# jhollowed/PyTEMDiags

Measured on AMD Instinct MI355X. Metric: grid-points/sec through full TEM pipeline (ncol*nlev*nt), higher is better.
Workload: dtype f64; 1 GPU; ne120 (777602 cols) x 72 lev x 30 snapshots per GPU, L=50, 1-degree zonal grid (M=180), ten GM16 Table-A1 outputs; ncol=777602, nlev=72, nt=30, sweeps=latitude-class, single sweep, mirror_paired_sweeps=True

## Files before the change

include/temx.h:

```cpp
#ifndef TEMX_H
#define TEMX_H

#include <stdint.h>

#ifdef __cplusplus
extern "C" {
#endif

typedef struct temx_plan temx_plan;

enum { TEMX_F64 = 0, TEMX_F32 = 1 };

enum {
  TEMX_OK = 0,
  TEMX_EINVAL = -1,
  TEMX_EHIP = -2,
  TEMX_ENOMEM = -3,
  TEMX_ERANK = -4,
  TEMX_ESTATE = -5,
  TEMX_EUNSUPPORTED = -6,
  TEMX_EINTERNAL = -7
};

enum {
  TEMX_DEFER_FINALIZE = 1,
  TEMX_NO_SYMMETRY = 2,
  TEMX_NO_CLASSES = 4,
  TEMX_NO_QR = 8,
  TEMX_LAT_TOL_F32 = 16
};

enum {
  TEMX_OPT_FORM = 1,
  TEMX_OPT_OS_MAP = 2,
  TEMX_OPT_OP_MAP = 3,
  TEMX_OPT_OS_SUBSAMPLE = 4,
  TEMX_OPT_TRACER_ONE_PASS = 5,
  TEMX_OPT_SINGLE_SWEEP_MIN_GROUPS = 6,
  TEMX_OPT_OS_CONTRACT = 7,
  TEMX_OPT_MISSING = 8,
  TEMX_OPT_MIN_COVERAGE = 9,
  TEMX_OPT_MISSING_WEIGHT = 10
};
enum {
  TEMX_FORM_AUTO = -1,
  TEMX_FORM_TWO_PASS = 0,
  TEMX_FORM_CLASS_SUMS = 1,
  TEMX_FORM_SINGLE_SWEEP = 2,
  TEMX_FORM_NO_SINGLE_SWEEP = 3,
  TEMX_FORM_MASKED = 4
};

enum {
  TEMX_MAT_Y0 = 0,
  TEMX_MAT_Y0P = 1,
  TEMX_MAT_GRAM = 2,
  TEMX_MAT_GINV = 3,
  TEMX_MAT_Y0INV = 4,
  TEMX_MAT_GRAM2 = 5,
  TEMX_MAT_GX = 6,
  TEMX_MAT_GSUB = 7,
  TEMX_MAT_COVERAGE = 8
};

enum {
// ... 135 lines not shown
```

pytemdiags_amd/_lib.py:

```python
from __future__ import annotations

import ctypes as C
import os

_HERE = os.path.dirname(os.path.abspath(__file__))
LIB_PATH = os.environ.get("TEMX_LIB") or os.path.join(_HERE, "libtemx.so")

ABI_VERSION = 402
F64, F32 = 0, 1
DEFER_FINALIZE = 1
NO_SYMMETRY = 2
NO_CLASSES = 4
NO_QR = 8
LAT_TOL_F32 = 16
MAT_Y0, MAT_Y0P, MAT_GRAM, MAT_GINV, MAT_Y0INV, MAT_GRAM2, MAT_GX, MAT_GSUB = 0, 1, 2, 3, 4, 5, 6, 7
MAT_COVERAGE = 8
OPT_FORM, OPT_OS_MAP, OPT_OP_MAP, OPT_OS_SUBSAMPLE, OPT_TRACER_ONE_PASS, OPT_SINGLE_SWEEP_MIN_GROUPS, OPT_OS_CONTRACT = 1, 2, 3, 4, 5, 6, 7
OPT_MISSING, OPT_MIN_COVERAGE, OPT_MISSING_WEIGHT = 8, 9, 10
MISSING_MODES = {"raise": 0, "mask": 1}
FORM_AUTO, FORM_TWO_PASS, FORM_CLASS_SUMS, FORM_SINGLE_SWEEP, FORM_NO_SINGLE_SWEEP = -1, 0, 1, 2, 3
FORM_MASKED = 4
FORMS = {"auto": FORM_AUTO, "two-pass": FORM_TWO_PASS, "class-sums": FORM_CLASS_SUMS,
         "single-sweep": FORM_SINGLE_SWEEP, "no-single-sweep": FORM_NO_SINGLE_SWEEP}

RESULT_NAMES = ("vtem", "omegatem", "wtem", "psitem", "epfy", "epfz", "epdiv",
                "utendepfd", "utendvtem", "utendwtem")
ZONAL_NAMES = ("ub", "vb", "thetab", "wapb", "upvpb", "upwappb", "vptpb", "dub_dp", "dthetab_dp",
               "ubcoslat", "dubcoslat_dlat", "psi", "psicoslat", "dpsicoslat_dlat", "dpsi_dp",
               "int_vbdp")
EDDY_NAMES = ("up", "vp", "thetap", "wapp", "upvp", "upwapp", "vptp")
TRACER_RESULT_NAMES = ("etfy", "etfz", "etdiv", "qtendetfd", "qtendvtem", "qtendwtem")
TRACER_ZONAL_NAMES = ("qb", "qpvpb", "qpwappb", "dqb_dp", "qbcoslat", "dqbcoslat_dlat")
TRACER_EDDY_NAMES = ("qp", "qpvp", "qpwapp")

ERRORS = {0: "TEMX_OK", -1: "TEMX_EINVAL", -2: "TEMX_EHIP", -3: "TEMX_ENOMEM", -4: "TEMX_ERANK",
          -5: "TEMX_ESTATE", -6: "TEMX_EUNSUPPORTED", -7: "TEMX_EINTERNAL"}

_vp, _i, _i64, _dp, _u64 = C.c_void_p, C.c_int, C.c_int64, C.POINTER(C.c_double), C.c_uint64
SIGNATURES = [
    ("temx_version", _i, []),
    ("temx_last_error", C.c_char_p, []),
# ... 100 lines not shown
```

pytemdiags_amd/csrc/kernels_op2.hpp:

```cpp
#pragma once
#include "kernels_op.hpp"

namespace temx {

template <int NA, int NB>
struct OpwSlot {
  double sd[2][NA][64];
  double y[NB * 16];
};

template <int TBS, int NA>
__device__ __forceinline__ void opw_round(const OpwSlot<NA, 2 * TBS>* slots, int par, int t0, int nbw,
                                          uint32_t yoff, int lane, double (&acc)[NA][(TBS + 1) / 2]) {
  asm volatile("s_waitcnt lgkmcnt(0)\n\ts_barrier" ::: "memory");
#pragma unroll
  for (int j = 0; j < 4; ++j) {
    double b[NA];
#pragma unroll
    for (int f = 0; f < NA; ++f) b[f] = slots[j].sd[par][f][lane];
#pragma unroll
    for (int tl = 0; tl < (TBS + 1) / 2; ++tl)
      if (tl < nbw) {
        const double ya = slots[j].y[(t0 + tl) * 16 + yoff];
#pragma unroll
// ... 554 lines not shown
};
template <> struct RowLoad<float> {
  static __device__ __forceinline__ void ld(float& dst, uint32_t voff, uint64_t sbase) {
    asm volatile("global_load_dword %0, %1, %2 " TEMX_ROWLOAD_MOD : "=v"(dst) : "v"(voff), "s"(sbase) : "memory");
  }
};
__device__ __forceinline__ double temx_rcp_count(double n) {
  double r = __builtin_amdgcn_rcp(n);
  return __builtin_fma(__builtin_fma(-n, r, 1.0), r, r);
}
template <int N, typename T>
__device__ __forceinline__ void row_wait(T& a, T& b, T& c, T& d) {
  asm volatile("s_waitcnt vmcnt(%4)" : "+v"(a), "+v"(b), "+v"(c), "+v"(d) : "n"(N) : "memory");
}
template <int N, typename T>
__device__ __forceinline__ void row_wait(T& a, T& b, T& c) {
  asm volatile("s_waitcnt vmcnt(%3)" : "+v"(a), "+v"(b), "+v"(c) : "n"(N) : "memory");
}
template <typename T>
__device__ __forceinline__ void row_touch(T& a) {
  asm volatile("" : "+v"(a)::"memory");
}

template <typename T, int TBS, int TBX, int NBR, int PD, int KIND = 0>
__global__ void __launch_bounds__(256, 1)
sweep_osr_kernel(FieldPtrs<4> fp, int64_t D, int K, int KX, const double* __restrict__ ycx,
                 const int4* __restrict__ crow, const int2* __restrict__ csplit,
                 const double* __restrict__ colscale, const double* __restrict__ rho, int K4,
                 double* __restrict__ px, double* __restrict__ pp, int nsplit, int ndt) {
  using KD = OsKind<KIND>;
  constexpr int NF = KD::NF, NFX = KD::NFX, NP = KD::NP;
  constexpr int NBX = 2 * TBX;
  constexpr int YE = NBX * 16;
  constexpr int YJ = (YE + 255) / 256;
  constexpr int MB = CLS_MB;
  constexpr int NCH = 4;
  constexpr int NV = 2 * (NF + NP);
  constexpr int NPR = KD::NPR, NPL = NP - NPR;
  static_assert(NBR <= TBS && TBS <= TBX, "reference degree <= L <= 2L");
  static_assert(YJ <= 2, "Y quarter per thread");
  static_assert((PD - 1) * CLS_MB * KD::NF + (CLS_MB - 1) * KD::NF + 2 <= 63, "the ring is counted in vmcnt (6 bits)");
  extern __shared__ double lds[];
  int split, dq;
  if (!wg_work((ndt + 3) / 4, nsplit, split, dq)) return;
  const int tid = threadIdx.x;
  const int wave = uniform_wave(), lane = tid & 63;
  const int c = lane & 15, g = lane >> 4;
  const int64_t colr = (int64_t)dq * 64 + lane < D ? (int64_t)dq * 64 + lane : D - 1;
  const uint32_t colb32 = (uint32_t)colr * (uint32_t)sizeof(T);
  const int dt = dq * 4 + wave;
  const int64_t d = (int64_t)dt * 16 + c;
  const bool dvalid = dt < ndt && d < D;
  const int64_t dcl = dvalid ? d : D - 1;
  const int b0 = __builtin_amdgcn_readfirstlane(csplit[split].x);
  const int b1 = __builtin_amdgcn_readfirstlane(csplit[split + 1].x);
  int grp = __builtin_amdgcn_readfirstlane(csplit[split].y);
  const uint32_t aoff_p = (uint32_t)(g * 4 + (lane & 3));
  const uint32_t aoff_r = (uint32_t)((lane & 3) * 4 + g);
  double* ybase = lds;
  double* cn = lds + 2 * YE;
  double* cb = lds + 2 * YE + 16 + wave * (NF * 2 * NBR * 64) + lane;
  double* apl = lds + 2 * YE + 16 + 4 * (NF * 2 * NBR * 64) + wave * (NPL * 2 * TBS * 64) + lane;
  double* ex = lds + 2 * YE + 16 + 4 * (NF * 2 * NBR * 64) + 4 * (NPL * 2 * TBS * 64);
  double* exw = ex + wave * 64 + lane;
  const double* exr = ex + g * 64 + wave * 16 + c;
  const double sth = (KD::TF >= 0 && colscale != nullptr) ? colscale[colr] : 1.0;
#pragma unroll
  for (int i = 0; i < NPL * 2 * TBS; ++i) apl[i * 64] = 0.0;
  double apr[NPR > 0 ? NPR : 1][2 * TBS];
#pragma unroll
  for (int k = 0; k < (NPR > 0 ? NPR : 1); ++k)
#pragma unroll
    for (int t = 0; t < 2 * TBS; ++t) apr[k][t] = 0.0;
#pragma unroll
  for (int f = 0; f < NF; ++f)
#pragma unroll
    for (int tb = 0; tb < 2 * NBR; ++tb) {
      const int l = tb < NBR ? 2 * (4 * tb + g) : 2 * (4 * (tb - NBR) + g) + 1;
      const double v = rho[((int64_t)f * K4 + (l < K ? l : K - 1)) * D + dcl];
      cb[(f * 2 * NBR + tb) * 64] = l < K ? v : 0.0;
    }
  uint64_t fbase[NF];
#pragma unroll
  for (int f = 0; f < NF; ++f) fbase[f] = reinterpret_cast<uint64_t>(fp.p[f]);
  { double sth_ready = sth; asm volatile("" : "+v"(sth_ready)); }

  double ax[NFX][NBX];
#pragma unroll
  for (int f = 0; f < NFX; ++f)
// ... 46 lines not shown
        const int ta = t < TBX ? tp : TBS + tp;
#pragma unroll
        for (int k = 0; k < NPR; ++k) apr[k][ta] = TEMX_MFMA4(ya, dP[k][t < TBX ? 0 : 1], apr[k][ta]);
        if constexpr (NPL > 0) {
          double v[NPL > 0 ? NPL : 1];
#pragma unroll
          for (int k = 0; k < NPL; ++k) v[k] = apl[(k * 2 * TBS + ta) * 64];
#pragma unroll
          for (int k = 0; k < NPL; ++k) v[k] = TEMX_MFMA4(ya, dP[NPR + k][t < TBX ? 0 : 1], v[k]);
#pragma unroll
          for (int k = 0; k < NPL; ++k) apl[(k * 2 * TBS + ta) * 64] = v[k];
        }
      }
    }
  };
  auto park_north = [&]() __attribute__((always_inline)) {
#pragma unroll
    for (int f = 0; f < NF; ++f) { sN[f] = s[f]; x0N[f] = x0[f]; s[f] = 0.0; }
#pragma unroll
    for (int k = 0; k < NP; ++k) { qN[k] = q[k]; q[k] = 0.0; }
    cntN = cnt;
    cnt = 0.0;
  };
  int4 rn;
  auto step = [&](auto posc, int b) __attribute__((always_inline)) {
    constexpr int POS = decltype(posc)::value % NCH;
    constexpr int P = decltype(posc)::value % PD;
    {
      const int4 r1 = rn;
      rn = crow[(int64_t)(b + PD) * 4 + wave];
      issue(std::integral_constant<int, (P + PD - 1) % PD>{}, r1);
    }
    if (left > 0) {
      if (!(TEMX_OS_SKIP & 1)) pending_chunk(std::integral_constant<int, POS>{});
      --left;
    }
    static_assert(NF == 4 || NF == 3, "row_wait has forms for 3 and 4 fields");
    static_for<MB>([&](auto jc) __attribute__((always_inline)) {
      constexpr int j = decltype(jc)::value;
      constexpr int NW = (PD - 1) * MB * NF + (MB - 1 - j) * NF;
      if constexpr (NF == 4) row_wait<NW>(xb[P][j][0], xb[P][j][1], xb[P][j][2], xb[P][j][3]);
      else row_wait<NW>(xb[P][j][0], xb[P][j][1], xb[P][j][2]);
    });
#pragma unroll
    for (int j = 0; j < YJ; ++j) row_touch(ys[j]);
    const int fl = er[P][0] >> 27;
    const bool south = (fl & (CLS_SOUTH << 1)) != 0;
    if ((fl & (CLS_FIRST << 1)) || (south && !prev_south)) {
      if (south && north_open) park_north();
      north_open = !south;
#pragma unroll
      for (int f = 0; f < NF; ++f) x0[f] = (double)xb[P][0][f];
    }
    prev_south = south;
#pragma unroll
    for (int j = 0; j < ((TEMX_OS_SKIP & 4) ? 0 : MB); ++j) {
      const double w = er[P][j] < 0 ? 0.0 : 1.0;
      double dx[NF];
#pragma unroll
      for (int f = 0; f < NF; ++f) dx[f] = (double)xb[P][j][f] - x0[f];
#pragma unroll
      for (int f = 0; f < NF; ++f) s[f] += w * dx[f];
#pragma unroll
      for (int k = 0; k < NP; ++k) q[k] += (w * dx[KD::pa(k)]) * dx[KD::pb(k)];
      cnt += w;
    }
    if (fl & (CLS_LAST << 1)) {
      prev_south = false;
      if (north_open) park_north();
      north_open = false;
      if (left > 0)
        static_for<NCH>([&](auto cc) __attribute__((always_inline)) {
          if (((decltype(cc)::value - POS - 1) & (NCH - 1)) < left) pending_chunk(cc);
        });
      const double rnN = cntN > 0.0 ? temx_rcp_count(cntN) : 0.0, rnS = cnt > 0.0 ? temx_rcp_count(cnt) : 0.0;
      double val[NV];
#pragma unroll
      for (int f = 0; f < NF; ++f) {
        const double sc = f == KD::TF ? sth : 1.0;
        val[f] = (sN[f] * rnN + x0N[f]) * sc;
        val[NF + NP + f] = (s[f] * rnS + x0[f]) * sc;
      }
#pragma unroll
      for (int k = 0; k < NP; ++k) {
        const double sc = k == KD::TP ? sth : 1.0;
        val[NF + k] = (qN[k] - sN[KD::pa(k)] * sN[KD::pb(k)] * rnN) * sc;
        val[2 * NF + NP + k] = (q[k] - s[KD::pa(k)] * s[KD::pb(k)] * rnS) * sc;
      }
      if (!(TEMX_OS_SKIP & 8)) asm volatile("s_waitcnt lgkmcnt(0)\n\ts_barrier" ::: "memory");
      ycur ^= 1;
      double* yw = ybase + ycur * YE;
#pragma unroll
      for (int v = 0; v < NV; ++v) exw[v * 256] = val[v];
      if (lane == 0) {
        cn[wave] = cntN;
        cn[4 + wave] = cnt;
      }
#pragma unroll
      for (int j = 0; j < YJ; ++j)
        if (tid + 256 * j < YE) yw[tid + 256 * j] = ys[j];
      if (!(TEMX_OS_SKIP & 8)) asm volatile("s_waitcnt lgkmcnt(0)\n\ts_barrier" ::: "memory");
      ++grp;
      load_ys(grp);
      double m2[2][NF], c2[2][NP];
#pragma unroll
      for (int f = 0; f < NF; ++f) {
        m2[0][f] = exr[f * 256];
        m2[1][f] = exr[(NF + NP + f) * 256];
      }
#pragma unroll
      for (int k = 0; k < NP; ++k) {
        c2[0][k] = exr[(NF + k) * 256];
        c2[1][k] = exr[(2 * NF + NP + k) * 256];
      }
      const double nN = cn[g], nS = cn[4 + g];
      double E[NF], O[NF];
#pragma unroll
      for (int f = 0; f < NF; ++f) E[f] = O[f] = 0.0;
#pragma unroll
      for (int tb = 0; tb < ((TEMX_OS_SKIP & 2) ? 0 : 2 * NBR); ++tb) {
        const int blk = tb < NBR ? tb : TBX + (tb - NBR);
        const double ya = yw[blk * 16 + aoff_r];
#pragma unroll
        for (int f = 0; f < NF; ++f) {
          if (tb < NBR)
            E[f] = TEMX_MFMA4(ya, cb[(f * 2 * NBR + tb) * 64], E[f]);
          else
            O[f] = TEMX_MFMA4(ya, cb[(f * 2 * NBR + tb) * 64], O[f]);
        }
      }
#pragma unroll
      for (int f = 0; f < NF; ++f) {
        m2[0][f] -= E[f] + O[f];
        m2[1][f] -= E[f] - O[f];
      }
#pragma unroll
      for (int f = 0; f < NFX; ++f) {
        const double SNf = nN * m2[0][f], SSf = nS * m2[1][f];
        dS[f][0] = SNf + SSf;
        dS[f][1] = SNf - SSf;
      }
#pragma unroll
      for (int k = 0; k < NP; ++k) {
        const double PNk = c2[0][k] + nN * m2[0][KD::pa(k)] * m2[0][KD::pb(k)];
        const double PSk = c2[1][k] + nS * m2[1][KD::pa(k)] * m2[1][KD::pb(k)];
        dP[k][0] = PNk + PSk;
        dP[k][1] = PNk - PSk;
      }
      yprev = yw;
      left = NCH;
#pragma unroll
      for (int f = 0; f < NF; ++f) s[f] = sN[f] = 0.0;
#pragma unroll
      for (int k = 0; k < NP; ++k) q[k] = qN[k] = 0.0;
      cnt = cntN = 0.0;
    }
  };

  if (b0 < b1) {
    load_ys(grp);
    rn = crow[(int64_t)b0 * 4 + wave];
    static_for<PD - 1>([&](auto kc) __attribute__((always_inline)) {
      constexpr int k = decltype(kc)::value;
      const int4 r0 = rn;
      rn = crow[(int64_t)(b0 + k + 1) * 4 + wave];
      issue(kc, r0);
    });
    constexpr int UNR = PD % 4 == 0 ? PD : PD % 2 == 0 ? 2 * PD : 4 * PD;
    for (int b = b0; b < b1; b += UNR)
      static_for<UNR>([&](auto kc) __attribute__((always_inline)) {
        constexpr int k = decltype(kc)::value;
        if (k == 0 || b + k < b1) step(kc, b + k);
      });
    asm volatile("s_waitcnt vmcnt(0)" ::: "memory");
  }
  if (left > 0) {
    const int first = (b1 - b0) & (NCH - 1);
    static_for<NCH>([&](auto cc) __attribute__((always_inline)) {
      if (((decltype(cc)::value - first) & (NCH - 1)) < left) pending_chunk(cc);
    });
  }
  if (dvalid) {
#pragma unroll
    for (int f = 0; f < NFX; ++f)
#pragma unroll
      for (int t = 0; t < NBX; ++t) {
        const int l = symx_harm<TBX>(t, g);
        if (l < (pp != nullptr ? KX : K4)) px[(((int64_t)split * NFX + f) * KX + l) * D + d] = ax[f][t];
      }
#pragma unroll
    for (int k = 0; k < NP; ++k)
#pragma unroll
      for (int t = 0; t < 2 * TBS; ++t) {
        const int l = sym_harm<TBS>(t, g);
        if (pp != nullptr && l < K) pp[(((int64_t)split * NP + k) * K + l) * D + d] = k < NPR ? apr[k < NPR ? k : 0][t] : apl[((k < NPR ? 0 : k - NPR) * 2 * TBS + t) * 64];
      }
  }
// ... 711 lines not shown
```

pytemdiags_amd/csrc/temx.hip:

```cpp
#include "../../include/temx.h"

#include <hip/hip_runtime.h>

#include <algorithm>
#include <cmath>
#include <cstdarg>
#include <cstdio>
#include <cstdlib>
#include <cstring>
#include <map>
#include <new>
#include <stdexcept>
#include <string>
#include <thread>
#include <atomic>
#include <vector>

#include "kernels.hpp"
#include "kernels_sym.hpp"
#include "kernels_cls.hpp"
#include "kernels_op.hpp"
#include "kernels_op2.hpp"
#include "kernels_osc.hpp"
#include "side_tables.hpp"
// ... 90 lines not shown
  int64_t cgroups = 0, cbatches = 0, ncls = 0;
  int64_t cls_max_side = 0;
  std::vector<int> gbatch0;
  DevBuf crow, ycls;
  std::map<int, DevBuf> csplits;
  Split sp_cproj4, sp_cproj1, sp_ceddy, sp_cflux;
  bool os_built = false, os_on = false;
  bool os_valid = false;
  DevBuf Axq, rho_t;
  int TBX = 0, KX = 0, KR = 0, NQ = 0;
  std::vector<double> h_xc, h_cnt;
  std::vector<int> h_crow;
  std::vector<int> sgbatch0;
  int64_t sgroups = 0, sbatches = 0;
  DevBuf ycx, ycx_s, crow_s, rho, rho0, gaunt , wq2, Gx, Gsinv, Ax , Axs ;
  std::vector<double> h_G_own;
  std::vector<double> h_Gx_own;
  std::vector<double> h_Gx, h_Gs;
  std::vector<double> h_T, h_Ginv, h_G, h_Yq;
  DevBuf oscblk, osAt, osAb, osAtq, osAbq, Bqp;
  OscMats osc{};
  bool osc_lds = false;
  int opt_os_contract = -1;
  int os_keep = 32;
  int64_t tD = 0, tnt = 0, tt0 = 0;
  int opt_form = -1, opt_os_map = -1, opt_op_map = -1, opt_tracer_one_pass = -1, opt_single_sweep_min_groups = -1;
  bool os_tile = false, op_tile = false;
  bool no_qr = false;
  DevBuf side_crow[2][2], side_gfirst[2][2];
  std::map<int, DevBuf> csplits_s;
  Split sp_os, sp_os_s;
  Split sp_copw;
  bool lcls = false, lone = false, xb_valid = false;
  DevBuf ycls_l, pbuf;
  int64_t ycls_lstride = 0;
  Split sp_lflux;
  bool onepass = false, op_valid = false;
  bool c4_valid = false;
  DevBuf csum, ccnt;
  DevBuf Pq;
  DevBuf csq, Pq2;
  bool tq_valid = false;
  DevBuf partial;
  DevBuf opB, opC;
  int opt_missing = 0, opt_min_cov = 500, opt_miss_w = 10;
  bool miss_built = false;
// ... 1442 lines not shown
      static std::atomic<uint64_t> attr_set{0};                                                                     \
      if (int rc_ = lds_attr_once(attr_set, pl->device, reinterpret_cast<const void*>(kern), (int)lds)) return rc_; \
      hipLaunchKernelGGL(kern, grid, block, lds, st, fp, pl->D, pl->K, pl->KX, sub ? pl->ycx_s.d() : pl->ycx.d(),   \
                         static_cast<const int4*>(sub ? pl->crow_s.p : pl->crow.p), cuts, pl->colscale.d(), rho,    \
                         pl->KR, px, pp, sp.nsplit, sp.ndt);                                                        \
      break;                                                                                                        \
    }                                                                                                               \
    if (sizeof(T) == 4) {                 \
      if (pl->cls_max_side > 8 * TEMX_F32_SIDE_CAP)                                                                 \
        return fail(TEMX_EUNSUPPORTED, "single sweep of fp32 fields: a latitude class of this plan has %lld members on one " \
                    "side, and the sweep sums a side in fp32; create the plan with TEMX_LAT_TOL_F32",               \
                    (long long)pl->cls_max_side);                                                                   \
      auto kern = sweep_os2_kernel<float, TBSv, TBXv, NBR, 2, KIND>;                                                \
      const size_t lds = ((size_t)2 * 2 * TBXv * 16 + 16 + (size_t)4 * KD::NF * 2 * NBR * 64 +                      \
                          (size_t)8 * (KD::NP - KD::NPR) * TBSv * 64 + (size_t)(KD::NF + KD::NP) * 512) * 8;        \
      static std::atomic<uint64_t> attr_set{0};                                                                     \
      if (int rc_ = lds_attr_once(attr_set, pl->device, reinterpret_cast<const void*>(kern), (int)lds)) return rc_; \
      const int si = sub ? 1 : 0;                                                                                   \
      hipLaunchKernelGGL(kern, grid, dim3(512), lds, st, fp, pl->D, pl->K, pl->KX, sub ? pl->ycx_s.d() : pl->ycx.d(), \
                         static_cast<const int4*>(pl->side_crow[si][0].p), static_cast<const int4*>(pl->side_crow[si][1].p), \
                         static_cast<const int*>(pl->side_gfirst[si][0].p), static_cast<const int*>(pl->side_gfirst[si][1].p), \
                         cuts, pl->colscale.d(), rho, pl->KR, px, pp, sp.nsplit, sp.ndt);                           \
    } else {                                                                                                        \
      auto kern = sweep_osr_kernel<double, TBSv, TBXv, NBR, 2, KIND>;                                               \
      const size_t lds = ((size_t)2 * 2 * TBXv * 16 + 16 + (size_t)4 * KD::NF * 2 * NBR * 64 +                      \
                          (size_t)4 * (KD::NP - KD::NPR) * 2 * TBSv * 64 + (size_t)2 * (KD::NF + KD::NP) * 256) * 8; \
      static std::atomic<uint64_t> attr_set{0};                                                                     \
      if (int rc_ = lds_attr_once(attr_set, pl->device, reinterpret_cast<const void*>(kern), (int)lds)) return rc_; \
      hipLaunchKernelGGL(kern, grid, block, lds, st, fp, pl->D, pl->K, pl->KX, sub ? pl->ycx_s.d() : pl->ycx.d(),   \
                         static_cast<const int4*>(sub ? pl->crow_s.p : pl->crow.p), cuts, pl->colscale.d(), rho,    \
                         pl->KR, px, pp, sp.nsplit, sp.ndt);                                                        \
    }                                                                                                               \
  } while (0)
  if (pl->TBS == 7 && pl->TBX == 13) TEMX_LOS(7, 13);
  else if (pl->TBS == 4 && pl->TBX == 8) TEMX_LOS(4, 8);
  else if (pl->TBS == 2 && pl->TBX == 4) TEMX_LOS(2, 4);
  else return fail(TEMX_EUNSUPPORTED, "single-sweep form: no instantiation for L = %d", pl->L);
#undef TEMX_LOS
  HIPCHK(hipGetLastError());
  return TEMX_OK;
}

template <int KIND>
static int launch_sweep_os(temx_plan* pl, const FieldPtrs<4>& fp, int dtype, bool sub, const double* rho, double* partial,
                           const Split& sp, hipStream_t st) {
  return dtype == TEMX_F64 ? launch_sweep_os_t<double, KIND>(pl, fp, sub, rho, partial, sp, st)
                           : launch_sweep_os_t<float, KIND>(pl, fp, sub, rho, partial, sp, st);
}

static bool os_supported(const temx_plan* pl) {
  if (!pl->cls || pl->large || pl->weighted || !pl->qbasis || pl->h_crow.empty()) return false;
  const int tbx = (pl->L + 1 + 3) / 4;
  return (pl->TBS == 7 && tbx <= 13) || (pl->TBS == 4 && tbx <= 8) || (pl->TBS == 2 && tbx <= 4);
}
// ... 473 lines not shown
  pl->TB = pl->K <= 16 ? 4 : (pl->K <= 32 ? 8 : (pl->K <= 52 ? 13 : 16));
  pl->stride = pl->TB;
  if (pl->K > 64) {
    pl->large = true;
    pl->nslice = (pl->K + 63) / 64;
    pl->stride = 16 * pl->nslice;
  }
  pl->K4 = 4 * pl->stride;
  pl->M = M;
  pl->lat_out_deg.assign(lat_out_deg_host, lat_out_deg_host + M);
  int rc = TEMX_OK;
  auto bail = [&](int code) {
    temx_plan_destroy(pl);
    return code;
  };

  const double d2r = M_PI / 180.0;
  std::vector<double> xs((size_t)std::max<int64_t>(ncol, M));
  for (int64_t i = 0; i < ncol; ++i) xs[i] = std::cos((90.0 - lat_deg_host[i]) * d2r);
  if ((rc = upload(pl->x, xs.data(), (size_t)ncol * 8))) return bail(rc);
  std::vector<double> norm((size_t)std::max(64, pl->K4), 0.0);
  for (int l = 0; l < pl->K; ++l) norm[l] = std::sqrt((2.0 * l + 1.0) / (4.0 * M_PI));
  if ((rc = upload(pl->norm, norm.data(), norm.size() * 8))) return bail(rc);
  int zero = 0;
  if ((rc = upload(pl->flag, &zero, sizeof(int)))) return bail(rc);

  if ((rc = pl->Y0.ensure((size_t)ncol * pl->K * 8))) return bail(rc);
  if ((rc = pl->yblk.ensure((size_t)(pl->nchunk + 1) * 4 * pl->stride * 16 * 8))) return bail(rc);
  if (hipMemset(pl->yblk.p, 0, pl->yblk.bytes) != hipSuccess) return bail(fail(TEMX_EHIP, "hipMemset of the Y0 blocks failed"));
  if ((rc = build_basis(pl, nullptr, nullptr, pl->Y0.d(), pl->yblk.d()))) return bail(rc);

  for (int m = 0; m < M; ++m) xs[m] = std::cos((90.0 - lat_out_deg_host[m]) * d2r);
  if ((rc = upload(pl->xo, xs.data(), (size_t)M * 8))) return bail(rc);
  if ((rc = pl->Y0p.ensure((size_t)M * pl->K * 8))) return bail(rc);
  if ((rc = pl->Qp.ensure((size_t)M * pl->K * 8))) return bail(rc);
  if ((rc = build_out_basis(pl, nullptr, pl->Y0p.d(), false))) return bail(rc);
  if ((rc = build_out_basis(pl, nullptr, pl->Qp.d(), true))) return bail(rc);

  {
    if ((rc = pl->G.ensure((size_t)pl->K * pl->K * 8))) return bail(rc);
    if ((rc = pl->Ginv.ensure((size_t)pl->K * pl->K * 8))) return bail(rc);
    Split sp = choose_split(pl->K, pl->nchunk, 2 * pl->num_cu);
    if ((rc = pl->partial.ensure((size_t)sp.nsplit * std::min(pl->K, 64) * pl->K * 8))) return bail(rc);
    FieldPtrs<1> fp;
    fp.p[0] = pl->Y0.p;
    if ((rc = project_all<1>(pl, fp, TEMX_F64, pl->K, nullptr, -1, sp, pl->G.d(), 0))) return bail(rc);
    hipError_t e = hipDeviceSynchronize();
    if (e != hipSuccess) return bail(fail(TEMX_EHIP, "gram kernel failed: %s", hipGetErrorString(e)));
// ... 369 lines not shown
struct FormChoice {
  bool two_pass;
  bool force_op;
  int os;
};
static FormChoice form_choice(const temx_plan* pl) {
  FormChoice c{false, false, -1};
  switch (pl->opt_form) {
    case TEMX_FORM_TWO_PASS: c.two_pass = true; c.os = 0; break;
    case TEMX_FORM_CLASS_SUMS: c.force_op = true; c.os = 0; break;
    case TEMX_FORM_SINGLE_SWEEP: c.force_op = true; c.os = 1; break;
    case TEMX_FORM_NO_SINGLE_SWEEP: c.os = 0; break;
    default: break;
  }
  if (const char* e = getenv("TEMX_TWO_PASS")) c.two_pass = e[0] == '1';
  if (const char* e = getenv("TEMX_ONE_PASS")) c.force_op = c.force_op || e[0] == '1';
  if (const char* e = getenv("TEMX_SINGLE_SWEEP")) c.os = e[0] == '0' ? 0 : (e[0] == '1' ? 1 : c.os);
  return c;
}
static bool tile_map(int opt, const char* env) {
  if (const char* e = getenv(env)) return !strcmp(e, "tile");
  return opt == 1;
}
static bool tracer_one_pass_wanted(const temx_plan* pl) {
  if (const char* e = getenv("TEMX_TRACER_ONE_PASS")) return e[0] == '1';
  return pl->opt_tracer_one_pass == 1;
}

int temx_plan_configure(temx_plan* pl, int option, int value) try {
  if (!pl) return fail(TEMX_EINVAL, "null plan");
  switch (option) {
    case TEMX_OPT_FORM:
      if (value < -1 || value > TEMX_FORM_NO_SINGLE_SWEEP) return fail(TEMX_EINVAL, "TEMX_OPT_FORM: unknown form %d", value);
      pl->opt_form = value;
      break;
    case TEMX_OPT_OS_MAP: pl->opt_os_map = value; break;
    case TEMX_OPT_OP_MAP: pl->opt_op_map = value; break;
    case TEMX_OPT_TRACER_ONE_PASS: pl->opt_tracer_one_pass = value; break;
    case TEMX_OPT_OS_SUBSAMPLE:
      if (value < 4) return fail(TEMX_EINVAL, "TEMX_OPT_OS_SUBSAMPLE: at least 4 class-groups");
      if (pl->os_built && value != pl->os_keep) return fail(TEMX_ESTATE, "the single-sweep tables of this plan are built: set the subsample before temx_plan_set_tem");
      pl->os_keep = value;
      break;
    case TEMX_OPT_SINGLE_SWEEP_MIN_GROUPS: pl->opt_single_sweep_min_groups = value; break;
    case TEMX_OPT_OS_CONTRACT: pl->opt_os_contract = value; break;
    case TEMX_OPT_MISSING:
      if (value != 0 && value != 1) return fail(TEMX_EINVAL, "TEMX_OPT_MISSING: 0 (raise) or 1 (mask), got %d", value);
      if (value == 1)
        if (int rc = miss_check(pl)) return rc;
      pl->opt_missing = value;
      pl->miss_valid = false;
      break;
    case TEMX_OPT_MIN_COVERAGE:
      if (value < 0 || value > 1000) return fail(TEMX_EINVAL, "TEMX_OPT_MIN_COVERAGE: per mille in 0..1000, got %d", value);
      pl->opt_min_cov = value;
      break;
    case TEMX_OPT_MISSING_WEIGHT:
      if (value < 4 || value > 14) return fail(TEMX_EINVAL, "TEMX_OPT_MISSING_WEIGHT: tau = 10^-value, value in 4..14, got %d", value);
      pl->opt_miss_w = value;
      break;
    default: return fail(TEMX_EINVAL, "unknown option %d", option);
  }
  pl->tem = false;
  return TEMX_OK;
} TEMX_CATCH

int temx_plan_option(const temx_plan* pl, int option) try {
  if (!pl) return -1;
  switch (option) {
    case TEMX_OPT_FORM:
      if (miss_mode(pl)) return TEMX_FORM_MASKED;
      return pl->os_on ? TEMX_FORM_SINGLE_SWEEP : ((pl->cls && pl->onepass) || (pl->lcls && pl->lone) ? TEMX_FORM_CLASS_SUMS : TEMX_FORM_TWO_PASS);
    case TEMX_OPT_OS_MAP: return tile_map(pl->opt_os_map, "TEMX_OS_MAP") ? 1 : 0;
    case TEMX_OPT_OP_MAP: return tile_map(pl->opt_op_map, "TEMX_OP_MAP") ? 1 : 0;
    case TEMX_OPT_TRACER_ONE_PASS: return tracer_one_pass_wanted(pl) ? 1 : 0;
    case TEMX_OPT_OS_SUBSAMPLE: return pl->os_keep;
    case TEMX_OPT_SINGLE_SWEEP_MIN_GROUPS: return pl->opt_single_sweep_min_groups;
    case TEMX_OPT_OS_CONTRACT: return pl->osc_lds ? 1 : 0;
    case TEMX_OPT_MISSING: return pl->opt_missing;
    case TEMX_OPT_MIN_COVERAGE: return pl->opt_min_cov;
    case TEMX_OPT_MISSING_WEIGHT: return pl->opt_miss_w;
    default: return -1;
  }
} TEMX_CATCH

int temx_plan_set_tem(temx_plan* pl, int nlev, int64_t nt, const double* p_pa_host, double p0) try {
  if (!pl || !p_pa_host) return fail(TEMX_EINVAL, "null argument");
  if (nlev < 2 || nt < 1) return fail(TEMX_EINVAL, "need nlev >= 2 and nt >= 1");
  if ((int64_t)nlev * nt >= ((int64_t)1 << 28)) return fail(TEMX_EINVAL, "nlev*nt must be < 2^28");
  if (pl->M < 2) return fail(TEMX_EINVAL, "need at least 2 zonal-mean latitudes");
  HIPCHK(hipSetDevice(pl->device));
  std::vector<double> p(p_pa_host, p_pa_host + nlev), tab;
  for (int j = 1; j < nlev; ++j)
    if (!(p[j] > p[j - 1])) return fail(TEMX_EINVAL, "pressure must be strictly ascending (front end flips)");
  pl->tem = false;
  pl->onepass = pl->lone = pl->op_valid = pl->xb_valid = pl->tq_valid = false;
  pl->os_on = pl->os_valid = false;
  pl->os_tile = tile_map(pl->opt_os_map, "TEMX_OS_MAP");
  {
    const char* e = getenv("TEMX_OS_CONTRACT");
    pl->osc_lds = e ? !strcmp(e, "lds") : pl->opt_os_contract == 1;
  }
  pl->op_tile = tile_map(pl->opt_op_map, "TEMX_OP_MAP");
  pl->nlev = nlev;
  pl->nt = nt;
  pl->D = (int64_t)nlev * nt;
  pl->tD = pl->D;
  pl->tnt = nt;
  pl->tt0 = 0;
  pl->p0 = p0;
  const int M = pl->M;
  const int64_t D = pl->D;
  int rc;
  if ((rc = upload(pl->p, p.data(), (size_t)nlev * 8))) return rc;
  gradient_table(p, tab);
  if ((rc = upload(pl->pg, tab.data(), tab.size() * 8))) return rc;
  std::vector<double> latr(M), cosl(M), fc(M);
  for (int m = 0; m < M; ++m) {
    const double lat = pl->lat_out_deg[m];
    latr[m] = lat * (M_PI / 180.0);
    cosl[m] = std::cos(lat * M_PI / 180.0);
    fc[m] = 2 * kOm * std::sin(lat * M_PI / 180.0);
  }
  gradient_table(latr, tab);
  if ((rc = upload(pl->lg, tab.data(), tab.size() * 8))) return rc;
  if ((rc = upload(pl->coslat, cosl.data(), (size_t)M * 8))) return rc;
// ... 924 lines not shown
  if (pl && miss_mode(pl)) return miss_refuse("temx_tracer_eddy");
  int rc = tem_ready(pl);
  if (rc) return rc;
  if (!q || !va || !wap || !ptrs3_host) return fail(TEMX_EINVAL, "null argument");
  if (!pl->Ct.p) return fail(TEMX_ESTATE, "temx_tracer_stage2 has not been called");
  HIPCHK(hipSetDevice(pl->device));
  if (!tail_is_whole(pl)) return fail(TEMX_ESTATE, "the plan holds the coefficients of a time slice (temx_tem_os_tail), not of the whole run");
  EddyOut eo{};
  eo.p[0] = ptrs3_host[0];
  eo.p[4] = ptrs3_host[1];
  eo.p[5] = ptrs3_host[2];
  if (unfused_stage2(pl)) {
    if (!pl->xb_valid) return fail(TEMX_ESTATE, "temx_tracer_stage2 has not been called since the last TEM run");
    return launch_eddy_from_xbar(pl, four(q, va, va, wap), dtype, native_means(pl, 4, 1, 1, 3), nullptr, eo,
                                 S_(stream));
  }
  return run_eddy<1>(pl, four(q, va, wap, nullptr), dtype, pl->Ct.d(), nullptr, &eo, S_(stream));
} TEMX_CATCH

int temx_status(temx_plan* pl, int* nonfinite, void* stream) try {
  if (!pl || !nonfinite) return fail(TEMX_EINVAL, "null argument");
  HIPCHK(hipSetDevice(pl->device));
  HIPCHK(hipStreamSynchronize(S_(stream)));
  int f = 0;
  HIPCHK(hipMemcpy(&f, pl->flag.p, sizeof(int), hipMemcpyDeviceToHost));
  *nonfinite = miss_mode(pl) ? 0 : f;
  if (f) {
    int zero = 0;
    HIPCHK(hipMemcpy(pl->flag.p, &zero, sizeof(int), hipMemcpyHostToDevice));
  }
  return TEMX_OK;
} TEMX_CATCH

int temx_synth_fields(int device, int64_t ncol, int nlev, int64_t nt, int64_t t0, const double* lat_deg,
                      const double* lon_deg, const double* plev_hpa, int dtype, uint64_t seed, void* ua,
                      void* va, void* ta, void* wap, void* stream) try {
  if (!lat_deg || !lon_deg || !plev_hpa || !ua || !va || !ta || !wap) return fail(TEMX_EINVAL, "null argument");
  HIPCHK(hipSetDevice(device));
  dim3 grid(256 * 16), block(256);
  if (dtype == TEMX_F64) {
    hipLaunchKernelGGL(synth_kernel<double>, grid, block, 0, S_(stream), ncol, nlev, nt, t0, lat_deg, lon_deg,
                       plev_hpa, seed, (double*)ua, (double*)va, (double*)ta, (double*)wap);
  } else if (dtype == TEMX_F32) {
    hipLaunchKernelGGL(synth_kernel<float>, grid, block, 0, S_(stream), ncol, nlev, nt, t0, lat_deg, lon_deg,
                       plev_hpa, seed, (float*)ua, (float*)va, (float*)ta, (float*)wap);
  } else {
    return fail(TEMX_EINVAL, "dtype must be TEMX_F64 or TEMX_F32");
  }
  HIPCHK(hipGetLastError());
  return TEMX_OK;
} TEMX_CATCH

int temx_mfma_f64_peak(int device, int iters, double* tflops_out) try {
// ... 70 lines not shown
```

pytemdiags_amd/engine.py:

```python
from __future__ import annotations

import ctypes as C

import numpy as np
import torch

from . import _lib
from ._lib import check

_DT = {torch.float64: _lib.F64, torch.float32: _lib.F32}


def _ptr(t):
    return C.c_void_p(t.data_ptr())


def _dbl(a):
    a = np.ascontiguousarray(a, dtype=np.float64)
    return a, a.ctypes.data_as(C.POINTER(C.c_double))


class Plan:

    def __init__(self, lat_deg, lat_out_deg, L, device=0, defer_finalize=False, symmetry=True, classes=True, qr=True,
# ... 21 lines not shown

    @property
    def paired(self):
        return bool(self.lib.temx_plan_is_paired(self._h))

    @property
    def sweep_mode(self):
        return int(self.lib.temx_plan_sweep_mode(self._h))

    @property
    def one_pass(self):
        return bool(self.lib.temx_plan_one_pass(self._h))

    @property
    def single_sweep(self):
        return bool(self.lib.temx_plan_single_sweep(self._h))

    @property
    def tracer_one_pass(self):
        return self.one_pass and self.option(_lib.OPT_TRACER_ONE_PASS) == 1

    def configure(self, form=None, os_map=None, op_map=None, os_subsample=None, tracer_one_pass=None,
                  single_sweep_min_groups=None, os_contract=None, missing=None, min_coverage=None,
                  missing_weight=None):
        def put(opt, val):
            check(self.lib.temx_plan_configure(self._h, opt, int(val)))
        if missing is not None:
            if missing not in _lib.MISSING_MODES:
                raise ValueError("missing must be 'raise' or 'mask', got %r" % (missing,))
            put(_lib.OPT_MISSING, _lib.MISSING_MODES[missing])
        if min_coverage is not None:
            mc = float(min_coverage)
            if not 0.0 <= mc <= 1.0:
                raise ValueError("min_coverage must lie in [0, 1], got %r" % (min_coverage,))
            put(_lib.OPT_MIN_COVERAGE, int(round(mc * 1000)))
        if missing_weight is not None:
            e = -np.log10(float(missing_weight))
            if not (float(missing_weight) > 0 and abs(e - round(e)) < 1e-9 and 4 <= round(e) <= 14):
                raise ValueError("missing_weight must be 10^-n with n in 4..14, got %r" % (missing_weight,))
            put(_lib.OPT_MISSING_WEIGHT, int(round(e)))
        if form is not None:
            put(_lib.OPT_FORM, _lib.FORMS[form] if isinstance(form, str) else form)
            self.form_requested = form
        for opt, val in ((_lib.OPT_OS_MAP, os_map), (_lib.OPT_OP_MAP, op_map)):
            if val is not None:
                put(opt, {"row": 0, "tile": 1}[val] if isinstance(val, str) else val)
        if os_subsample is not None:
            put(_lib.OPT_OS_SUBSAMPLE, os_subsample)
        if tracer_one_pass is not None:
            put(_lib.OPT_TRACER_ONE_PASS, 1 if tracer_one_pass else 0)
        if single_sweep_min_groups is not None:
            put(_lib.OPT_SINGLE_SWEEP_MIN_GROUPS, single_sweep_min_groups)
        if os_contract is not None:
            put(_lib.OPT_OS_CONTRACT, {"mfma": 0, "lds": 1}[os_contract] if isinstance(os_contract, str) else os_contract)
        self.nlev = self.nt = self.D = None

    def option(self, opt):
        return int(self.lib.temx_plan_option(self._h, int(opt)))

    @property
    def missing(self):
        return "mask" if self.option(_lib.OPT_MISSING) == 1 else "raise"

    def coverage(self):
        D = getattr(self, "_cov_D", None) or self.D or 1
        out = torch.empty((self.M, D), dtype=torch.float64, device=self.device)
        check(self.lib.temx_get_matrix(self._h, _lib.MAT_COVERAGE, _ptr(out), self._stream()))
        return out

    def close(self):
        if getattr(self, "_h", None) is not None and self._h.value:
            self.lib.temx_plan_destroy(self._h)
            self._h = C.c_void_p()

    def __del__(self):
        try:
            self.close()
# ... 405 lines not shown
```

Before: 177.9 billion grid-points/s.

## Replace single-sweep workgroup barriers with LDS counter handoff between waves

In the single-sweep kernel, the two s_barrier points at each latitude-group boundary are replaced by per-wave LDS atomic counters. The tile contraction (tile_role) is deferred into the next step, so waves can keep issuing loads and draining pending chunks instead of stalling at a full workgroup barrier. A bounded spin-wait with a failure flag reports a timeout through temx_status, and the old barrier form stays selectable through an option or environment variable. This adds spin-polling overhead and ordering risk, since the waits use relaxed atomics.

```diff
diff --git a/include/temx.h b/include/temx.h
--- a/include/temx.h
+++ b/include/temx.h
@@ -40,7 +40,8 @@
   TEMX_OPT_OS_CONTRACT = 7,
   TEMX_OPT_MISSING = 8,
   TEMX_OPT_MIN_COVERAGE = 9,
-  TEMX_OPT_MISSING_WEIGHT = 10
+  TEMX_OPT_MISSING_WEIGHT = 10,
+  TEMX_OPT_OS_SYNC = 11
 };
 enum {
   TEMX_FORM_AUTO = -1,
diff --git a/pytemdiags_amd/_lib.py b/pytemdiags_amd/_lib.py
--- a/pytemdiags_amd/_lib.py
+++ b/pytemdiags_amd/_lib.py
@@ -17,6 +17,7 @@
 MAT_COVERAGE = 8
 OPT_FORM, OPT_OS_MAP, OPT_OP_MAP, OPT_OS_SUBSAMPLE, OPT_TRACER_ONE_PASS, OPT_SINGLE_SWEEP_MIN_GROUPS, OPT_OS_CONTRACT = 1, 2, 3, 4, 5, 6, 7
 OPT_MISSING, OPT_MIN_COVERAGE, OPT_MISSING_WEIGHT = 8, 9, 10
+OPT_OS_SYNC = 11
 MISSING_MODES = {"raise": 0, "mask": 1}
 FORM_AUTO, FORM_TWO_PASS, FORM_CLASS_SUMS, FORM_SINGLE_SWEEP, FORM_NO_SINGLE_SWEEP = -1, 0, 1, 2, 3
 FORM_MASKED = 4
diff --git a/pytemdiags_amd/csrc/kernels_op2.hpp b/pytemdiags_amd/csrc/kernels_op2.hpp
--- a/pytemdiags_amd/csrc/kernels_op2.hpp
+++ b/pytemdiags_amd/csrc/kernels_op2.hpp
@@ -600,12 +600,16 @@
   asm volatile("" : "+v"(a)::"memory");
 }
 
-template <typename T, int TBS, int TBX, int NBR, int PD, int KIND = 0>
+constexpr int HANDOFF_LOOKS = 1 << 22;
+__device__ __forceinline__ uint32_t handoff_look(const uint32_t* ctr) {
+  return __hip_atomic_load(ctr, __ATOMIC_RELAXED, __HIP_MEMORY_SCOPE_WORKGROUP);
+}
+template <typename T, int TBS, int TBX, int NBR, int PD, int KIND = 0, int SYNC = 0>
 __global__ void __launch_bounds__(256, 1)
 sweep_osr_kernel(FieldPtrs<4> fp, int64_t D, int K, int KX, const double* __restrict__ ycx,
                  const int4* __restrict__ crow, const int2* __restrict__ csplit,
                  const double* __restrict__ colscale, const double* __restrict__ rho, int K4,
-                 double* __restrict__ px, double* __restrict__ pp, int nsplit, int ndt) {
+                 double* __restrict__ px, double* __restrict__ pp, int nsplit, int ndt, int* __restrict__ hstat) {
   using KD = OsKind<KIND>;
   constexpr int NF = KD::NF, NFX = KD::NFX, NP = KD::NP;
   constexpr int NBX = 2 * TBX;
@@ -642,7 +646,12 @@
   double* ex = lds + 2 * YE + 16 + 4 * (NF * 2 * NBR * 64) + 4 * (NPL * 2 * TBS * 64);
   double* exw = ex + wave * 64 + lane;
   const double* exr = ex + g * 64 + wave * 16 + c;
+  uint32_t* hctr = reinterpret_cast<uint32_t*>(ex + NV * 256);
   const double sth = (KD::TF >= 0 && colscale != nullptr) ? colscale[colr] : 1.0;
+  if constexpr (SYNC != 0) {
+    if (tid < 2) hctr[tid] = 0u;
+    __syncthreads();
+  }
 #pragma unroll
   for (int i = 0; i < NPL * 2 * TBS; ++i) apl[i * 64] = 0.0;
   double apr[NPR > 0 ? NPR : 1][2 * TBS];
@@ -735,14 +744,97 @@
     cntN = cnt;
     cnt = 0.0;
   };
+  auto tile_role = [&](const double* yw) __attribute__((always_inline)) {
+    double m2[2][NF], c2[2][NP];
+#pragma unroll
+    for (int f = 0; f < NF; ++f) {
+      m2[0][f] = exr[f * 256];
+      m2[1][f] = exr[(NF + NP + f) * 256];
+    }
+#pragma unroll
+    for (int k = 0; k < NP; ++k) {
+      c2[0][k] = exr[(NF + k) * 256];
+      c2[1][k] = exr[(2 * NF + NP + k) * 256];
+    }
+    const double nN = cn[g], nS = cn[4 + g];
+    double E[NF], O[NF];
+#pragma unroll
+    for (int f = 0; f < NF; ++f) E[f] = O[f] = 0.0;
+#pragma unroll
+    for (int tb = 0; tb < ((TEMX_OS_SKIP & 2) ? 0 : 2 * NBR); ++tb) {
+      const int blk = tb < NBR ? tb : TBX + (tb - NBR);
+      const double ya = yw[blk * 16 + aoff_r];
+#pragma unroll
+      for (int f = 0; f < NF; ++f) {
+        if (tb < NBR)
+          E[f] = TEMX_MFMA4(ya, cb[(f * 2 * NBR + tb) * 64], E[f]);
+        else
+          O[f] = TEMX_MFMA4(ya, cb[(f * 2 * NBR + tb) * 64], O[f]);
+      }
+    }
+    if constexpr (SYNC != 0) {
+      asm volatile("s_waitcnt lgkmcnt(0)" ::: "memory");
+      if (lane == 0) __hip_atomic_fetch_add(&hctr[1], 1u, __ATOMIC_RELAXED, __HIP_MEMORY_SCOPE_WORKGROUP);
+    }
+#pragma unroll
+    for (int f = 0; f < NF; ++f) {
+      m2[0][f] -= E[f] + O[f];
+      m2[1][f] -= E[f] - O[f];
+    }
+#pragma unroll
+    for (int f = 0; f < NFX; ++f) {
+      const double SNf = nN * m2[0][f], SSf = nS * m2[1][f];
+      dS[f][0] = SNf + SSf;
+      dS[f][1] = SNf - SSf;
+    }
+#pragma unroll
+    for (int k = 0; k < NP; ++k) {
+      const double PNk = c2[0][k] + nN * m2[0][KD::pa(k)] * m2[0][KD::pb(k)];
+      const double PSk = c2[1][k] + nS * m2[1][KD::pa(k)] * m2[1][KD::pb(k)];
+      dP[k][0] = PNk + PSk;
+      dP[k][1] = PNk - PSk;
+    }
+    yprev = yw;
+    left = NCH;
+  };
+  uint32_t hgen = 0;
+  bool hpend = false;
+  int hfail = 0;
+  const double* ypend = ybase;
+  auto handoff_wait = [&](const uint32_t* ctr, uint32_t seen, uint32_t need, int code) __attribute__((always_inline)) {
+    seen = (uint32_t)__builtin_amdgcn_readfirstlane((int)seen);
+    if (seen >= need || hfail != 0) return;
+#pragma unroll 1
+    for (int n = 0; n < HANDOFF_LOOKS; ++n) {
+      __builtin_amdgcn_s_sleep(1);
+      seen = (uint32_t)__builtin_amdgcn_readfirstlane((int)handoff_look(ctr));
+      if (seen >= need) return;
+    }
+    hfail = code;
+  };
   int4 rn;
   auto step = [&](auto posc, int b) __attribute__((always_inline)) {
     constexpr int POS = decltype(posc)::value % NCH;
     constexpr int P = decltype(posc)::value % PD;
+    uint32_t seen = 0;
+    if constexpr (SYNC != 0) {
+      if (hpend) seen = handoff_look(&hctr[0]);
+    }
     {
       const int4 r1 = rn;
       rn = crow[(int64_t)(b + PD) * 4 + wave];
       issue(std::integral_constant<int, (P + PD - 1) % PD>{}, r1);
+    }
+    if constexpr (SYNC != 0) {
+      if (hpend) {
+        if (left > 0)
+          static_for<NCH>([&](auto cc) __attribute__((always_inline)) {
+            if (((decltype(cc)::value - POS) & (NCH - 1)) < left) pending_chunk(cc);
+          });
+        handoff_wait(&hctr[0], seen, 4u * hgen, 1);
+        tile_role(ypend);
+        hpend = false;
+      }
     }
     if (left > 0) {
       if (!(TEMX_OS_SKIP & 1)) pending_chunk(std::integral_constant<int, POS>{});
@@ -782,10 +874,15 @@
       prev_south = false;
       if (north_open) park_north();
       north_open = false;
-      if (left > 0)
-        static_for<NCH>([&](auto cc) __attribute__((always_inline)) {
-          if (((decltype(cc)::value - POS - 1) & (NCH - 1)) < left) pending_chunk(cc);
-        });
+      uint32_t seen_done = 0;
+      if constexpr (SYNC == 0) {
+        if (left > 0)
+          static_for<NCH>([&](auto cc) __attribute__((always_inline)) {
+            if (((decltype(cc)::value - POS - 1) & (NCH - 1)) < left) pending_chunk(cc);
+          });
+      } else {
+        seen_done = handoff_look(&hctr[1]);
+      }
       const double rnN = cntN > 0.0 ? temx_rcp_count(cntN) : 0.0, rnS = cnt > 0.0 ? temx_rcp_count(cnt) : 0.0;
       double val[NV];
 #pragma unroll
@@ -800,7 +897,11 @@
         val[NF + k] = (qN[k] - sN[KD::pa(k)] * sN[KD::pb(k)] * rnN) * sc;
         val[2 * NF + NP + k] = (q[k] - s[KD::pa(k)] * s[KD::pb(k)] * rnS) * sc;
       }
-      if (!(TEMX_OS_SKIP & 8)) asm volatile("s_waitcnt lgkmcnt(0)\n\ts_barrier" ::: "memory");
+      if constexpr (SYNC == 0) {
+        if (!(TEMX_OS_SKIP & 8)) asm volatile("s_waitcnt lgkmcnt(0)\n\ts_barrier" ::: "memory");
+      } else {
+        handoff_wait(&hctr[1], seen_done, 4u * hgen, 2);
+      }
       ycur ^= 1;
       double* yw = ybase + ycur * YE;
 #pragma unroll
@@ -812,56 +913,18 @@
 #pragma unroll
       for (int j = 0; j < YJ; ++j)
         if (tid + 256 * j < YE) yw[tid + 256 * j] = ys[j];
-      if (!(TEMX_OS_SKIP & 8)) asm volatile("s_waitcnt lgkmcnt(0)\n\ts_barrier" ::: "memory");
+      if constexpr (SYNC == 0) {
+        if (!(TEMX_OS_SKIP & 8)) asm volatile("s_waitcnt lgkmcnt(0)\n\ts_barrier" ::: "memory");
+      } else {
+        asm volatile("s_waitcnt lgkmcnt(0)" ::: "memory");
+        if (lane == 0) __hip_atomic_fetch_add(&hctr[0], 1u, __ATOMIC_RELAXED, __HIP_MEMORY_SCOPE_WORKGROUP);
+        ++hgen;
+        hpend = true;
+        ypend = yw;
+      }
       ++grp;
       load_ys(grp);
-      double m2[2][NF], c2[2][NP];
-#pragma unroll
-      for (int f = 0; f < NF; ++f) {
-        m2[0][f] = exr[f * 256];
-        m2[1][f] = exr[(NF + NP + f) * 256];
-      }
-#pragma unroll
-      for (int k = 0; k < NP; ++k) {
-        c2[0][k] = exr[(NF + k) * 256];
-        c2[1][k] = exr[(2 * NF + NP + k) * 256];
-      }
-      const double nN = cn[g], nS = cn[4 + g];
-      double E[NF], O[NF];
-#pragma unroll
-      for (int f = 0; f < NF; ++f) E[f] = O[f] = 0.0;
-#pragma unroll
-      for (int tb = 0; tb < ((TEMX_OS_SKIP & 2) ? 0 : 2 * NBR); ++tb) {
-        const int blk = tb < NBR ? tb : TBX + (tb - NBR);
-        const double ya = yw[blk * 16 + aoff_r];
-#pragma unroll
-        for (int f = 0; f < NF; ++f) {
-          if (tb < NBR)
-            E[f] = TEMX_MFMA4(ya, cb[(f * 2 * NBR + tb) * 64], E[f]);
-          else
-            O[f] = TEMX_MFMA4(ya, cb[(f * 2 * NBR + tb) * 64], O[f]);
-        }
-      }
-#pragma unroll
-      for (int f = 0; f < NF; ++f) {
-        m2[0][f] -= E[f] + O[f];
-        m2[1][f] -= E[f] - O[f];
-      }
-#pragma unroll
-      for (int f = 0; f < NFX; ++f) {
-        const double SNf = nN * m2[0][f], SSf = nS * m2[1][f];
-        dS[f][0] = SNf + SSf;
-        dS[f][1] = SNf - SSf;
-      }
-#pragma unroll
-      for (int k = 0; k < NP; ++k) {
-        const double PNk = c2[0][k] + nN * m2[0][KD::pa(k)] * m2[0][KD::pb(k)];
-        const double PSk = c2[1][k] + nS * m2[1][KD::pa(k)] * m2[1][KD::pb(k)];
-        dP[k][0] = PNk + PSk;
-        dP[k][1] = PNk - PSk;
-      }
-      yprev = yw;
-      left = NCH;
+      if constexpr (SYNC == 0) tile_role(yw);
 #pragma unroll
       for (int f = 0; f < NF; ++f) s[f] = sN[f] = 0.0;
 #pragma unroll
@@ -886,6 +949,19 @@
         if (k == 0 || b + k < b1) step(kc, b + k);
       });
     asm volatile("s_waitcnt vmcnt(0)" ::: "memory");
+  }
+  if constexpr (SYNC != 0) {
+    if (hpend) {
+      if (left > 0) {
+        const int first = (b1 - b0) & (NCH - 1);
+        static_for<NCH>([&](auto cc) __attribute__((always_inline)) {
+          if (((decltype(cc)::value - first) & (NCH - 1)) < left) pending_chunk(cc);
+        });
+      }
+      handoff_wait(&hctr[0], handoff_look(&hctr[0]), 4u * hgen, 1);
+      tile_role(ypend);
+    }
+    if (hfail != 0 && lane == 0) atomicOr(hstat, hfail);
   }
   if (left > 0) {
     const int first = (b1 - b0) & (NCH - 1);
diff --git a/pytemdiags_amd/csrc/temx.hip b/pytemdiags_amd/csrc/temx.hip
--- a/pytemdiags_amd/csrc/temx.hip
+++ b/pytemdiags_amd/csrc/temx.hip
@@ -136,6 +136,8 @@
   OscMats osc{};
   bool osc_lds = false;
   int opt_os_contract = -1;
+  bool os_barrier = false;
+  int opt_os_sync = -1;
   int os_keep = 32;
   int64_t tD = 0, tnt = 0, tt0 = 0;
   int opt_form = -1, opt_os_map = -1, opt_op_map = -1, opt_tracer_one_pass = -1, opt_single_sweep_min_groups = -1;
@@ -1624,14 +1626,17 @@
                          static_cast<const int*>(pl->side_gfirst[si][0].p), static_cast<const int*>(pl->side_gfirst[si][1].p), \
                          cuts, pl->colscale.d(), rho, pl->KR, px, pp, sp.nsplit, sp.ndt);                           \
     } else {                                                                                                        \
-      auto kern = sweep_osr_kernel<double, TBSv, TBXv, NBR, 2, KIND>;                                               \
-      const size_t lds = ((size_t)2 * 2 * TBXv * 16 + 16 + (size_t)4 * KD::NF * 2 * NBR * 64 +                      \
-                          (size_t)4 * (KD::NP - KD::NPR) * 2 * TBSv * 64 + (size_t)2 * (KD::NF + KD::NP) * 256) * 8; \
-      static std::atomic<uint64_t> attr_set{0};                                                                     \
-      if (int rc_ = lds_attr_once(attr_set, pl->device, reinterpret_cast<const void*>(kern), (int)lds)) return rc_; \
+       \
+      constexpr size_t lds = ((size_t)2 * 2 * TBXv * 16 + 16 + (size_t)4 * KD::NF * 2 * NBR * 64 +                  \
+                              (size_t)4 * (KD::NP - KD::NPR) * 2 * TBSv * 64 + (size_t)2 * (KD::NF + KD::NP) * 256 + 2) * 8; \
+      static_assert(lds <= 163840, "the single sweep's workgroup fits the LDS of a compute unit");                 \
+      auto kern = pl->os_barrier ? sweep_osr_kernel<double, TBSv, TBXv, NBR, 2, KIND, 0>                            \
+                                 : sweep_osr_kernel<double, TBSv, TBXv, NBR, 2, KIND, 1>;                           \
+      static std::atomic<uint64_t> attr_set[2] = {{0}, {0}};                                                        \
+      if (int rc_ = lds_attr_once(attr_set[pl->os_barrier ? 0 : 1], pl->device, reinterpret_cast<const void*>(kern), (int)lds)) return rc_; \
       hipLaunchKernelGGL(kern, grid, block, lds, st, fp, pl->D, pl->K, pl->KX, sub ? pl->ycx_s.d() : pl->ycx.d(),   \
                          static_cast<const int4*>(sub ? pl->crow_s.p : pl->crow.p), cuts, pl->colscale.d(), rho,    \
-                         pl->KR, px, pp, sp.nsplit, sp.ndt);                                                        \
+                         pl->KR, px, pp, sp.nsplit, sp.ndt, static_cast<int*>(pl->flag.p) + 1);                     \
     }                                                                                                               \
   } while (0)
   if (pl->TBS == 7 && pl->TBX == 13) TEMX_LOS(7, 13);
@@ -2151,8 +2156,8 @@
   std::vector<double> norm((size_t)std::max(64, pl->K4), 0.0);
   for (int l = 0; l < pl->K; ++l) norm[l] = std::sqrt((2.0 * l + 1.0) / (4.0 * M_PI));
   if ((rc = upload(pl->norm, norm.data(), norm.size() * 8))) return bail(rc);
-  int zero = 0;
-  if ((rc = upload(pl->flag, &zero, sizeof(int)))) return bail(rc);
+  const int zero[2] = {0, 0};
+  if ((rc = upload(pl->flag, zero, sizeof(zero)))) return bail(rc);
 
   if ((rc = pl->Y0.ensure((size_t)ncol * pl->K * 8))) return bail(rc);
   if ((rc = pl->yblk.ensure((size_t)(pl->nchunk + 1) * 4 * pl->stride * 16 * 8))) return bail(rc);
@@ -2568,6 +2573,10 @@
   if (const char* e = getenv(env)) return !strcmp(e, "tile");
   return opt == 1;
 }
+static bool os_barrier_wanted(const temx_plan* pl) {
+  if (const char* e = getenv("TEMX_OS_SYNC")) return !strcmp(e, "barrier");
+  return pl->opt_os_sync == 1;
+}
 static bool tracer_one_pass_wanted(const temx_plan* pl) {
   if (const char* e = getenv("TEMX_TRACER_ONE_PASS")) return e[0] == '1';
   return pl->opt_tracer_one_pass == 1;
@@ -2605,6 +2614,10 @@
       if (value < 4 || value > 14) return fail(TEMX_EINVAL, "TEMX_OPT_MISSING_WEIGHT: tau = 10^-value, value in 4..14, got %d", value);
       pl->opt_miss_w = value;
       break;
+    case TEMX_OPT_OS_SYNC:
+      if (value != 0 && value != 1) return fail(TEMX_EINVAL, "TEMX_OPT_OS_SYNC: 0 (flags) or 1 (barriers), got %d", value);
+      pl->opt_os_sync = value;
+      break;
     default: return fail(TEMX_EINVAL, "unknown option %d", option);
   }
   pl->tem = false;
@@ -2626,6 +2639,7 @@
     case TEMX_OPT_MISSING: return pl->opt_missing;
     case TEMX_OPT_MIN_COVERAGE: return pl->opt_min_cov;
     case TEMX_OPT_MISSING_WEIGHT: return pl->opt_miss_w;
+    case TEMX_OPT_OS_SYNC: return os_barrier_wanted(pl) ? 1 : 0;
     default: return -1;
   }
 } TEMX_CATCH
@@ -2648,6 +2662,7 @@
     pl->osc_lds = e ? !strcmp(e, "lds") : pl->opt_os_contract == 1;
   }
   pl->op_tile = tile_map(pl->opt_op_map, "TEMX_OP_MAP");
+  pl->os_barrier = os_barrier_wanted(pl);
   pl->nlev = nlev;
   pl->nt = nt;
   pl->D = (int64_t)nlev * nt;
@@ -3618,13 +3633,17 @@
   if (!pl || !nonfinite) return fail(TEMX_EINVAL, "null argument");
   HIPCHK(hipSetDevice(pl->device));
   HIPCHK(hipStreamSynchronize(S_(stream)));
-  int f = 0;
-  HIPCHK(hipMemcpy(&f, pl->flag.p, sizeof(int), hipMemcpyDeviceToHost));
+  int fw[2] = {0, 0};
+  HIPCHK(hipMemcpy(fw, pl->flag.p, sizeof(fw), hipMemcpyDeviceToHost));
+  const int f = fw[0];
   *nonfinite = miss_mode(pl) ? 0 : f;
-  if (f) {
-    int zero = 0;
-    HIPCHK(hipMemcpy(pl->flag.p, &zero, sizeof(int), hipMemcpyHostToDevice));
-  }
+  if (f || fw[1]) {
+    const int zero[2] = {0, 0};
+    HIPCHK(hipMemcpy(pl->flag.p, zero, sizeof(zero), hipMemcpyHostToDevice));
+  }
+  if (fw[1])
+    return fail(TEMX_EINTERNAL, "single sweep: the hand-over of the class sums between the waves of a workgroup timed out "
+                "(code %d); results of the runs since the last temx_status are invalid. TEMX_OS_SYNC=barrier selects the barrier form", fw[1]);
   return TEMX_OK;
 } TEMX_CATCH
 
diff --git a/pytemdiags_amd/engine.py b/pytemdiags_amd/engine.py
--- a/pytemdiags_amd/engine.py
+++ b/pytemdiags_amd/engine.py
@@ -67,7 +67,7 @@
 
     def configure(self, form=None, os_map=None, op_map=None, os_subsample=None, tracer_one_pass=None,
                   single_sweep_min_groups=None, os_contract=None, missing=None, min_coverage=None,
-                  missing_weight=None):
+                  missing_weight=None, os_sync=None):
         def put(opt, val):
             check(self.lib.temx_plan_configure(self._h, opt, int(val)))
         if missing is not None:
@@ -98,6 +98,8 @@
             put(_lib.OPT_SINGLE_SWEEP_MIN_GROUPS, single_sweep_min_groups)
         if os_contract is not None:
             put(_lib.OPT_OS_CONTRACT, {"mfma": 0, "lds": 1}[os_contract] if isinstance(os_contract, str) else os_contract)
+        if os_sync is not None:
+            put(_lib.OPT_OS_SYNC, {"flags": 0, "barrier": 1}[os_sync] if isinstance(os_sync, str) else os_sync)
         self.nlev = self.nt = self.D = None
 
     def option(self, opt):
```

After: 188.3 billion grid-points/s, median of 6. 1.06x the previous value.
